# JosefAlbers/Phi-3-Vision-MLX

Measured on AMD Instinct MI355X. Metric: decode tokens/sec through generate()'s loop (reference-defined; bare graph replays: device_rate) + prefill ms, Phi-3-Vision bf16 1-image VQA, higher is better.
Workload: dtype bf16; 1 GPU; Phi-3-Vision single 336x336 image VQA (BASELINE configs[1]); 17 crops, 2509 image tokens + 22 text tokens, prompt 2531, B=1 per GPU, greedy, EOS suppressed; parallelism=batch-sharded replicas x1, batch_per_gpu=1, tiny=False

## Files before the change

### include/p3v.h

```cpp
#ifndef P3V_H
#define P3V_H
#include <stdint.h>

#ifdef __cplusplus
extern "C" {
#endif

#define P3V_VERSION 600
#define P3V_OK 0
#define P3V_ERR_ARG (-22)
#define P3V_ERR_LAUNCH (-5)
#define P3V_ERR_UNSUPPORTED (-95)
#define P3V_ERR_HIP (-14)

typedef struct {
  int cu_count, lds_per_cu, wave_size, clock_khz, mem_clock_khz, mem_bus_bits;
  int64_t hbm_bytes;
  char arch[32];
} p3v_props_t;

int p3v_version(void);
int p3v_device_props(int device, p3v_props_t* out );
const char* p3v_strerror(int code);

// ... 24 lines not shown
  const uint16_t* W;
  void* out;
  const uint16_t* bias;
  const void* resid;
  const uint16_t* pos;
  int M, N, K;
  int lda, ldw, ldo;
  int epilogue;
  int patches_per_img;
  void* ws;
  int64_t ws_bytes;
} p3v_gemm_args_t;
int p3v_gemm(const p3v_gemm_args_t* args , void* stream);
int64_t p3v_gemm_ws_bytes(int M, int N, int K, int epilogue);
int p3v_gemm_rows_slices(int M, int N, int K, int epilogue);

typedef struct {
  const uint16_t* x;
  const uint16_t* W;
  void* out;
  const uint16_t* resid;
  const uint16_t* norm_w;
  float norm_eps;
  int M, N, K;
  int epilogue;
} p3v_gemv_args_t;
int p3v_gemv(const p3v_gemv_args_t* args , void* stream);

typedef struct {
  const uint16_t* x; const uint8_t* W; const float* w_scale; void* out;
// ... 327 lines not shown
```

### phi-3-vision-mlx_amd/_lib.py

```python
import ctypes as C
import os

_HERE = os.path.dirname(os.path.abspath(__file__))
LIB_PATH = os.environ.get("P3V_LIB") or os.path.join(_HERE, "libp3v.so")

P3V_OK = 0
(EPI_NONE, EPI_BIAS, EPI_BIAS_QGELU, EPI_BIAS_GELU, EPI_BIAS_RESID_F32, EPI_RESID_BF16, EPI_SILU_MUL, EPI_PATCH,
 EPI_F32) = range(9)
DECODE_MAX_L = 16

vp, i32, i64, f32 = C.c_void_p, C.c_int, C.c_int64, C.c_float


class Props(C.Structure):
    _fields_ = [("cu_count", i32), ("lds_per_cu", i32), ("wave_size", i32), ("clock_khz", i32),
                ("mem_clock_khz", i32), ("mem_bus_bits", i32), ("hbm_bytes", i64), ("arch", C.c_char * 32)]


class GemmArgs(C.Structure):
    _fields_ = [("A", vp), ("W", vp), ("out", vp), ("bias", vp), ("resid", vp), ("pos", vp),
                ("M", i32), ("N", i32), ("K", i32), ("lda", i32), ("ldw", i32), ("ldo", i32),
                ("epilogue", i32), ("patches_per_img", i32), ("ws", vp), ("ws_bytes", i64)]


# ... 143 lines not shown
SAMPLE_MAX_N, SAMPLE_MAX_ROWS = 32768, 1024
POOL_LAST, POOL_MEAN = 0, 1
SIM_TOPK_MAX, SIM_TOPK_MAX_Q = 32, 16
SIGNATURES = {
    "p3v_version": (i32, []),
    "p3v_device_props": (i32, [i32, C.POINTER(Props)]),
    "p3v_strerror": (C.c_char_p, [i32]),
    "p3v_set_tuning": (i32, [C.c_char_p, i32]),
    "p3v_get_tuning": (i32, [C.c_char_p, C.POINTER(i32)]),
    "p3v_embed_gather": (i32, [vp, vp, vp, i32, i32, i32, vp]),
    "p3v_rmsnorm": (i32, [vp, vp, vp, i32, i32, f32, vp]),
    "p3v_layernorm": (i32, [vp, vp, vp, vp, i32, i32, i32, f32, vp]),
    "p3v_gemm": (i32, [C.POINTER(GemmArgs), vp]),
    "p3v_gemm_ws_bytes": (i64, [i32, i32, i32, i32]),
    "p3v_gemm_rows_slices": (i32, [i32, i32, i32, i32]),
    "p3v_gemv": (i32, [C.POINTER(GemvArgs), vp]),
    "p3v_gemv_step": (i32, [C.POINTER(GemvArgs), C.POINTER(GemvStep), vp]),
    "p3v_gemv_fp8_step": (i32, [C.POINTER(GemvF8Args), C.POINTER(GemvStep), vp]),
    "p3v_gemv_q4_step": (i32, [C.POINTER(GemvQ4Args), C.POINTER(GemvStep), vp]),
    "p3v_gemv_fp8": (i32, [C.POINTER(GemvF8Args), vp]),
    "p3v_dequant_fp8": (i32, [vp, vp, vp, i32, i32, vp]),
    "p3v_pack_b13": (i32, [vp, i32, i32, i32, vp, vp, vp]),
    "p3v_unpack_b13": (i32, [vp, i32, i32, i32, i32, vp, vp]),
    "p3v_gemv_b13": (i32, [C.POINTER(GemvB13Args), vp]),
    "p3v_gemv_b13_plan": (i32, [i32, i32, i32, i32, C.POINTER(i32)]),
    "p3v_gemv_b13_step": (i32, [C.POINTER(GemvB13Args), C.POINTER(GemvStep), vp]),
    "p3v_gemm_fp8": (i32, [C.POINTER(GemmF8Args), vp]),
    "p3v_quant_fp8_rows": (i32, [vp, vp, f32, vp, vp, i32, i32, vp]),
    "p3v_rope_table": (i32, [vp, vp, f32, vp, vp, i32, i32, vp]),
    "p3v_rope_kv_append": (i32, [vp, vp, vp, vp, vp, vp, i32, i32, i32, i32, i32, i32, vp, i32, i32, i32, i32, f32, vp]),
# ... 88 lines not shown
```

### phi-3-vision-mlx_amd/csrc/p3v_common.h

```cpp
#pragma once
#include <hip/hip_runtime.h>
#include <stdint.h>

#include "../../include/p3v.h"

typedef uint16_t bf16_t;
typedef __attribute__((ext_vector_type(8))) __bf16 bf16x8_t;
typedef __attribute__((ext_vector_type(4))) float f32x4_t;
typedef __attribute__((ext_vector_type(16))) float f32x16_t;
typedef __attribute__((ext_vector_type(4))) uint32_t u32x4_t;
typedef __attribute__((ext_vector_type(2))) uint32_t u32x2_t;

#define P3V_WAVE 64
#define P3V_MAX_DEVICES 64

#define P3V_CHECK_LAUNCH()                                   \
  do {                                                       \
    hipError_t e_ = hipGetLastError();                       \
    if (e_ != hipSuccess) return P3V_ERR_LAUNCH;             \
  } while (0)

__device__ __forceinline__ float bf16_to_f32(bf16_t u) { return __uint_as_float(((uint32_t)u) << 16); }

typedef __attribute__((ext_vector_type(2))) __bf16 bf16x2_t;
// ... 84 lines not shown
  float t = -INFINITY;
  for (int i = 0; i < nw; ++i) t = fmaxf(t, red[i]);
  return t;
}

static inline int p3v_cdiv(long a, long b) { return (int)((a + b - 1) / b); }
static inline int p3v_gemv_wpw(int waves, int n_cu, int forced) {
  if (forced == 3 || forced == 4) return forced;
  const float w3 = (float)p3v_cdiv(p3v_cdiv(waves, 3), n_cu) * 3.f * n_cu / (float)waves;
  const float w4 = (float)p3v_cdiv(p3v_cdiv(waves, 4), n_cu) * 4.f * n_cu / (float)waves;
  return w3 < w4 - 0.05f ? 3 : 4;
}

struct P3vTuning {
  int gemm_big_rows;
  int gemm_no_splitk, gemm_splitk_max_m, gemm_splitk_max_s, gemm_splitk_wgs, gemm_128, gemm_persistent;
  int gemm_rows;
  int gemm_no_skinny, gemm_skinny_max_m, gemm_skinny_s, gemm_skinny_tm128;
  int gemm_no_qkv_fuse;
  int gemm_f8_narrow;
  int attn_no_dma, attn_old, attn_pp, attn_il, attn_il_waves, combine_g, kvq_old, q8_old;
  int attn_fo_map_q8;
  int attn_fo_map;
  int gemv_no_mfma, gemv_no_mfma8, gemv_wpc, gemv8_wgs, gemv_variant, gemv_rows, gemv8_min, gemv_mfma8, gemv_f8_wpc, gemv_q4_wpc, gemv_wpw, gemv_q4_rows_wgs, gemv_q4_rows8;
  int gemv_b13_wpc, gemv_b13_wpc_end;
  int gemv_b13_xscale;
};
const P3vTuning& p3v_tuning();
```

### phi-3-vision-mlx_amd/csrc/p3v_gemm.hip

```cpp
#include <stdlib.h>
#include <string.h>


#include "p3v_gemm_qkv.h"

#define P3V_EPI_QKV 100

#define BM 128
#define BN 128
#define BK 64
#define TILE_BYTES (BM * BK * 2)
#define GEMM_LDS (4 * TILE_BYTES)

typedef const __attribute__((address_space(1))) void* gptr_t;
typedef __attribute__((address_space(3))) void* lptr_t;

struct GemmP {
  const bf16_t* A; const bf16_t* W; void* out; const bf16_t* bias; const void* resid; const bf16_t* pos;
  int M, N, K, lda, ldw, ldo, ppi;
  int kslice;
  QkvP q;
};

__device__ __forceinline__ float gelu_erf(float x) { return 0.5f * x * (1.f + erff(x * 0.70710678118654752f)); }
// ... 242 lines not shown
  if (!attr_set) {
    if (hipFuncSetAttribute((const void*)k_gemm<EPI, ORD>, hipFuncAttributeMaxDynamicSharedMemorySize, GEMM_LDS) != hipSuccess)
      return P3V_ERR_HIP;
    attr_set = true;
  }
  const int n_tile = EPI == P3V_EPI_SILU_MUL ? BN / 2 : BN;
  dim3 grid(p3v_cdiv(p.N, n_tile), p3v_cdiv(p.M, BM), p.kslice ? p.K / p.kslice : 1);
  hipLaunchKernelGGL((k_gemm<EPI, ORD>), grid, dim3(256), GEMM_LDS, s, p);
  P3V_CHECK_LAUNCH();
  return P3V_OK;
}

template <int EPI>
static int launch_gemm(const GemmP& p, hipStream_t s) { return launch_gemm_v<EPI, 0>(p, s); }

int p3v_gemm256_try(const p3v_gemm_args_t* a, hipStream_t s);
static int gemm128(const p3v_gemm_args_t* a, hipStream_t s);

static int gemm_big_rows(const p3v_gemm_args_t* a) {
  const int n_big = a->epilogue == P3V_EPI_SILU_MUL ? 128 : 256, n_small = n_big / 2;
  if (a->M < 1024 || a->N % n_big || a->epilogue == P3V_EPI_PATCH) return 0;
  if (const int force = p3v_tuning().gemm_big_rows; force >= 0) return min(force / 256 * 256, a->M);
  const int mt = p3v_cdiv(a->M, 256), nt_big = a->N / n_big, nt_small = p3v_cdiv(a->N, n_small);
  const float big_round = a->K >= 2048 ? 1.0f : 1.0f + 0.25f * (2048 - a->K) / 1024.f;
  float best = 1e30f;
  int best_rows = 0;
  for (int ms = 0; ms <= mt; ++ms) {
    const int rows_big = min(ms * 256, a->M), rows_small = a->M - rows_big;
    const long big = (long)ms * nt_big, small = (long)p3v_cdiv(rows_small, 128) * nt_small;
    float c = (float)((big + 255) / 256) * big_round;
    if (small) {
      const long full = small / 512, rest = small % 512;
      c += 0.675f * full + (rest == 0 ? 0.f : rest <= 256 ? 0.42f : 0.675f);
    }
    if (big && small) c += 0.04f;
    if (c < best - 1e-4f) { best = c; best_rows = rows_big; }
  }
  return best_rows;
}

template <int EPI>
__global__ void __launch_bounds__(256) k_splitk_reduce(const float* __restrict__ part, void* __restrict__ out, const void* __restrict__ resid,
                                                       int M, int N, int ldp, int ldo, int S) {
  constexpr bool SILU = EPI == P3V_EPI_SILU_MUL;
  const int per_row = N / 8;
  const long i = (long)blockIdx.x * 256 + threadIdx.x;
  if (i >= (long)M * per_row) return;
  const int m = (int)(i / per_row), n = (int)(i - (long)m * per_row) * 8;
  float v[8] = {0, 0, 0, 0, 0, 0, 0, 0}, u[8] = {0, 0, 0, 0, 0, 0, 0, 0};
  for (int z = 0; z < S; ++z) {
    const float* pr = part + ((size_t)z * M + m) * ldp + n;
    const float4 a0 = *(const float4*)pr, a1 = *(const float4*)(pr + 4);
    v[0] += a0.x; v[1] += a0.y; v[2] += a0.z; v[3] += a0.w; v[4] += a1.x; v[5] += a1.y; v[6] += a1.z; v[7] += a1.w;
// ... 152 lines not shown
  if (a->M == 0) return P3V_OK;
  {
    const size_t w_rows = (size_t)a->N * (a->epilogue == P3V_EPI_SILU_MUL ? 2 : 1);
    if ((size_t)a->M * a->lda * 2 >= (1ull << 32) || w_rows * a->ldw * 2 >= (1ull << 32)) return P3V_ERR_UNSUPPORTED;
  }
  hipStream_t s = (hipStream_t)stream;
  if (!a->bias) {
    const int rc = p3v_gemm_skinny_try(a, s);
    if (rc != P3V_ERR_UNSUPPORTED) return rc;
  }
  {
    const int rc = gemm_splitk(a, s);
    if (rc != P3V_ERR_UNSUPPORTED) return rc;
  }
  const bool big_tiles = !p3v_tuning().gemm_128;
  const int rows_big = big_tiles ? gemm_big_rows(a) : 0;
  if (rows_big > 0) {
    p3v_gemm_args_t top = *a;
    top.M = rows_big;
    const int rc = p3v_gemm256_try(&top, s);
    if (rc == P3V_OK && rows_big < a->M) {
      const bool f32_out = a->epilogue == P3V_EPI_BIAS_RESID_F32 || a->epilogue == P3V_EPI_F32;
      const size_t out_row = (size_t)a->ldo * (f32_out ? 4 : 2);
      p3v_gemm_args_t rest = *a;
      rest.M = a->M - rows_big;
      rest.A = a->A + (size_t)rows_big * a->lda;
      rest.out = (char*)a->out + rows_big * out_row;
      if (a->resid) rest.resid = (const char*)a->resid + rows_big * out_row;
      return gemm128(&rest, s);
    }
    if (rc != P3V_ERR_UNSUPPORTED) return rc;
  }
  return gemm128(a, s);
}

// ... 25 lines not shown
  if (sp->B <= 0 || sp->L <= 0 || nh <= 0 || nkv <= 0 || hd <= 0 || sp->tab_div <= 0 || !(sp->q_scale > 0.f)) return P3V_ERR_ARG;
  if (a->M != sp->B * sp->L || a->N != (nh + 2 * nkv) * hd || a->K % BK || a->lda < a->K || a->ldw < a->K || a->lda % 8 || a->ldw % 8) return P3V_ERR_ARG;
  if (((uintptr_t)a->A | (uintptr_t)a->W | (uintptr_t)a->bias | (uintptr_t)sp->q_out | (uintptr_t)sp->k_dst | (uintptr_t)sp->v_dst |
       (uintptr_t)sp->cos_t | (uintptr_t)sp->sin_t) & 15)
    return P3V_ERR_ARG;
  const int dpos0 = sp->dst_off_is_past ? sp->past : 0;
  if (hd % 32 || half % 16 || dpos0 % 8 || sp->dst_t % 8 || p3v_tuning().gemm_no_qkv_fuse) return P3V_ERR_UNSUPPORTED;
  if ((size_t)a->M * a->lda * 2 >= (1ull << 32) || (size_t)a->N * a->ldw * 2 >= (1ull << 32)) return P3V_ERR_UNSUPPORTED;
  hipStream_t s = (hipStream_t)stream;
  QkvP q = {sp->cos_t, sp->sin_t, sp->q_out, sp->k_dst, sp->v_dst, sp->L, nh, nkv, hd, sp->past, dpos0, sp->dst_t, sp->tab_t, sp->tab_div, 0,
            sp->q_scale};
  if (a->M < 1024) return p3v_gemm_skinny_qkv(a, q, s);
  if ((nh * hd) % BN || (nkv * hd) % BN || p3v_tuning().gemm_128) return P3V_ERR_UNSUPPORTED;
  p3v_gemm_args_t plain = *a;
  plain.epilogue = P3V_EPI_NONE;
  int rows_big = (nh * hd) % 256 || (nkv * hd) % 256 ? 0 : gemm_big_rows(&plain);
  if (rows_big > 0) {
    p3v_gemm_args_t top = *a;
    top.M = rows_big;
    const int rc = p3v_gemm256_qkv(&top, q, s);
    if (rc == P3V_ERR_UNSUPPORTED) rows_big = 0;
    else if (rc != P3V_OK) return rc;
  }
  if (rows_big < a->M) {
    q.m_base = rows_big;
    const GemmP p = {a->A + (size_t)rows_big * a->lda, a->W, nullptr, a->bias, nullptr, nullptr, a->M - rows_big, a->N, a->K, a->lda, a->ldw, 0, 0, 0, q};
    return launch_gemm<P3V_EPI_QKV>(p, s);
  }
  return P3V_OK;
}
```

### phi-3-vision-mlx_amd/csrc/p3v_gemm256.hip

```cpp
#include <stdlib.h>

#include "p3v_gemm256_epi.h"

#define BUF_BYTES (4 * HALF_BYTES)
#define GEMM256_LDS (2 * BUF_BYTES)

struct Tile256 {
  int m0, n0; int a_off[2][2], b_off[2][2]; __amdgpu_buffer_rsrc_t rs_a;
  int swapped, is_k, row0;
};

#ifdef P3V_G256_DEBUG
__device__ unsigned long long p3v_g256dbg[8 * 64 * 8];
#define G_S(k) do { __builtin_amdgcn_sched_barrier(0); asm volatile("s_memtime %0" : "=s"(g_s[k])); __builtin_amdgcn_sched_barrier(0); } while (0)
#define G_FLUSH(it) do { if (blockIdx.x == P3V_G256_DEBUG && (threadIdx.x & 63) == 0 && (it) < 64) { for (int k_ = 0; k_ < 8; ++k_) p3v_g256dbg[((threadIdx.x >> 6) * 64 + (it)) * 8 + k_] = g_s[k_]; } } while (0)
extern "C" int p3v_g256dbg_read(unsigned long long* out) {
  return hipMemcpyFromSymbol(out, HIP_SYMBOL(p3v_g256dbg), sizeof(unsigned long long) * 8 * 64 * 8) == hipSuccess ? 0 : -1;
}
#else
#define G_S(k) do { } while (0)
#define G_FLUSH(it) do { } while (0)
#endif
template <int EPI, int SCHED = 0x50, int ORDER = 0>
__global__ void __launch_bounds__(512, 1) k_gemm256(Gemm256P p) {
  constexpr bool SILU = EPI == P3V_EPI_SILU_MUL, QKV = EPI == P3V_EPI_QKV;
  extern __shared__ __attribute__((aligned(16))) unsigned char smem[];
  const int tid = threadIdx.x, lane = tid & 63, wave = __builtin_amdgcn_readfirstlane(tid >> 6);
  const int wr = wave >> 2, wc = wave & 3;
  constexpr int n_out_tile = SILU ? TN / 2 : TN;
  const int gx = (p.N + n_out_tile - 1) / n_out_tile, gy = (p.M + TM - 1) / TM, nwg = gx * gy;
  const int nq_t = QKV ? p.q.nh * p.q.hd / TN : 0, nk_t = QKV ? p.q.nkv * p.q.hd / TN : 0;

  using Tile = Tile256;
  const int srow = tid >> 3, schunk = tid & 7;
  auto make_tile = [&](int wid, Tile& t) {
    const int q = nwg >> 3, r = nwg & 7, xcd = wid & 7, loc = wid >> 3;
    const int id = (xcd < r ? xcd * (q + 1) : r * (q + 1) + (xcd - r) * q) + loc;
    constexpr int BAND = 4;
    const int band = id / (BAND * gx), in_band = id % (BAND * gx);
    const int rows = min(BAND, gy - band * BAND);
    const int m_t = band * BAND + in_band % rows, n_t = in_band / rows;
    t.m0 = m_t * TM, t.n0 = n_t * n_out_tile;
    t.swapped = t.is_k = t.row0 = 0;
    if (QKV) {
      t.swapped = n_t >= nq_t + nk_t;
      t.is_k = !t.swapped && n_t >= nq_t;
      t.row0 = t.swapped ? (p.q.nh + p.q.nkv) * p.q.hd : t.is_k ? p.q.nh * p.q.hd : 0;
      t.n0 = (n_t - (t.swapped ? nq_t + nk_t : t.is_k ? nq_t : 0)) * TN;
    }
#pragma unroll
    for (int h = 0; h < 2; ++h)
#pragma unroll
      for (int qq = 0; qq < 2; ++qq) {
        const int rr = h * 128 + qq * 64 + srow;
        const int sw = (schunk ^ (rr & 7)) * 8;
        const int ar = min(t.m0 + rr, p.M - 1) - t.m0;
        int br;
        if (SILU) {
          const int wcol = rr >> 6, ni = (rr & 63) >> 4, c = rr & 15;
          br = min(t.n0 + wcol * 32 + (ni & 1) * 16 + c, p.N - 1) + (ni >> 1) * p.N;
        } else if (QKV) {
          br = qkv_pair_row(p.q, t.row0, t.n0 >> 1, rr);
        } else {
          br = min(t.n0 + rr, p.N - 1);
        }
        if (QKV && t.swapped) {
          t.a_off[h][qq] = (rr * p.ldw + sw) * 2;
          t.b_off[h][qq] = (int)(((unsigned)(t.m0 + ar) * (unsigned)p.lda + (unsigned)sw) * 2u);
        } else {
          t.a_off[h][qq] = (ar * p.lda + sw) * 2;
          t.b_off[h][qq] = (int)(((unsigned)br * (unsigned)p.ldw + (unsigned)sw) * 2u);
        }
      }
    t.rs_a = QKV && t.swapped ? __builtin_amdgcn_make_buffer_rsrc((void*)(p.W + (size_t)(t.row0 + t.n0) * p.ldw), 0, 0xffffffff, 0x00020000)
                              : __builtin_amdgcn_make_buffer_rsrc((void*)(p.A + (size_t)t.m0 * p.lda), 0, 0xffffffff, 0x00020000);
  };
  const __amdgpu_buffer_rsrc_t rs_w = __builtin_amdgcn_make_buffer_rsrc((void*)p.W, 0, 0xffffffff, 0x00020000);
  const __amdgpu_buffer_rsrc_t rs_x = __builtin_amdgcn_make_buffer_rsrc((void*)p.A, 0, 0xffffffff, 0x00020000);
  auto dma_half = [&](const Tile& t, int which, int kt, int buf) {
    unsigned char* base = smem + buf * BUF_BYTES + which * HALF_BYTES + wave * 1024;
    const int h = which & 1;
#pragma unroll
    for (int q = 0; q < 2; ++q) {
      const __amdgpu_buffer_rsrc_t rs = which < 2 ? t.rs_a : (QKV && t.swapped) ? rs_x : rs_w;
      const int vo = which < 2 ? t.a_off[h][q] : t.b_off[h][q];
      __builtin_amdgcn_raw_ptr_buffer_load_lds(rs, (lptr_t)(base + q * 8192), 16, vo, kt * (TK * 2), 0, 0);
    }
  };

  const int frow = lane & 15, fchunk = lane >> 4;
  const int nk = p.K / TK;
  int wid = blockIdx.x;
  if (wid >= nwg) return;
  Tile cur_t;
  make_tile(wid, cur_t);
#pragma unroll
  for (int w4 = 0; w4 < 4; ++w4) dma_half(cur_t, w4, 0, 0);
  int gk = 0;
  bool landed = false;
  for (;;) {
  const int m0 = cur_t.m0, n0 = cur_t.n0;
  const bool has_next = wid + (int)gridDim.x < nwg;
  f32x4_t acc[8][4];
#pragma unroll
  for (int i = 0; i < 8; ++i)
#pragma unroll
    for (int j = 0; j < 4; ++j) acc[i][j] = (f32x4_t){0.f, 0.f, 0.f, 0.f};

#ifdef P3V_G256_DEBUG
  unsigned long long g_s[8] = {0, 0, 0, 0, 0, 0, 0, 0};
#endif
  for (int kt = 0; kt < nk; ++kt, ++gk) {
    G_S(0);
    if (!(kt == 0 && landed)) asm volatile("s_waitcnt vmcnt(0)" ::: "memory");
    G_S(1);
    __builtin_amdgcn_s_barrier();
    G_S(2);
    const bool last = kt + 1 == nk;
    const bool more = !last || has_next;
    const int nb = (gk + 1) & 1;
    const unsigned char* ta = smem + (gk & 1) * BUF_BYTES + wr * HALF_BYTES;
    const unsigned char* tb = smem + (gk & 1) * BUF_BYTES + (2 + (wc >> 1)) * HALF_BYTES + (wc & 1) * 64 * 128;
    bf16x8_t af[4][2], af1[4][2], bf0[2][2], bf1[2][2];
    auto read_a_to = [&](int sub, bf16x8_t (&dst)[4][2]) {
#pragma unroll
      for (int i = 0; i < 4; ++i)
#pragma unroll
        for (int kk = 0; kk < 2; ++kk) {
          const int r = sub * 64 + i * 16 + frow;
          dst[i][kk] = *(const bf16x8_t*)(ta + r * 128 + (((kk * 4 + fchunk) ^ (r & 7)) << 4));
        }
    };
    auto read_a = [&](int sub) { read_a_to(sub, af); };
    auto read_b = [&](int sub, bf16x8_t (&bf)[2][2]) {
#pragma unroll
      for (int j = 0; j < 2; ++j)
#pragma unroll
        for (int kk = 0; kk < 2; ++kk) {
          const int r = sub * 32 + j * 16 + frow;
          bf[j][kk] = *(const bf16x8_t*)(tb + r * 128 + (((kk * 4 + fchunk) ^ (r & 7)) << 4));
        }
    };
    auto quad_from = [&](int asub, int bsub, bf16x8_t (&a)[4][2], bf16x8_t (&bf)[2][2]) {
      __builtin_amdgcn_s_setprio(1);
#pragma unroll
      for (int kk = 0; kk < 2; ++kk)
#pragma unroll
        for (int i = 0; i < 4; ++i)
#pragma unroll
          for (int j = 0; j < 2; ++j)
            acc[asub * 4 + i][bsub * 2 + j] =
                __builtin_amdgcn_mfma_f32_16x16x32_bf16(bf[j][kk], a[i][kk], acc[asub * 4 + i][bsub * 2 + j], 0, 0, 0);
      __builtin_amdgcn_s_setprio(0);
    };
    auto quad = [&](int asub, int bsub, bf16x8_t (&bf)[2][2]) { quad_from(asub, bsub, af, bf); };
    auto dma_phase = [&](int ph) {
      if (more) {
#pragma unroll
        for (int h = 0; h < 4; ++h)
          if (((SCHED >> (2 * h)) & 3) == ph) {
            if (!last) dma_half(cur_t, h, kt + 1, nb);
            else {
              Tile nt;
              make_tile(wid + gridDim.x, nt);
              dma_half(nt, h, 0, nb);
            }
          }
// ... 35 lines not shown
    read_a(1);
    if (ORDER == 1) dma_phase(2);
    quad(1, 1, bf1);
    dma_phase(3);
    quad(1, 0, bf0);
  }

  if (has_next) {
    asm volatile("s_waitcnt vmcnt(0)" ::: "memory");
    landed = true;
  }
  if constexpr (QKV) {
    if (!cur_t.swapped) qkv_epilogue_rot<8>(p.q, acc, p.bias, cur_t.is_k, cur_t.row0, (n0 >> 1) + wc * 32, m0 + wr * 128, p.M, lane);
    else qkv_epilogue_vt<8>(p.q, acc, p.bias ? p.bias + cur_t.row0 : nullptr, n0 + wr * 128, m0 + wc * 64, p.M, lane);
  } else {
    gemm256_epilogue<EPI>(p, acc, m0, n0, wr, wc, lane);
  }
  if (!has_next) break;
  wid += gridDim.x;
  make_tile(wid, cur_t);
  }
}

template <int EPI, int SCHED, int ORDER>
static int launch_gemm256_v(const Gemm256P& p, hipStream_t s) {
  static bool attr_set = false;
  if (!attr_set) {
    if (hipFuncSetAttribute((const void*)k_gemm256<EPI, SCHED, ORDER>, hipFuncAttributeMaxDynamicSharedMemorySize, GEMM256_LDS) != hipSuccess)
      return P3V_ERR_HIP;
    attr_set = true;
  }
  const int n_tile = EPI == P3V_EPI_SILU_MUL ? TN / 2 : TN;
  static int n_cu = 0;
  if (!n_cu) {
    int dev = 0;
    hipDeviceProp_t pr;
    if (hipGetDevice(&dev) != hipSuccess || hipGetDeviceProperties(&pr, dev) != hipSuccess) return P3V_ERR_HIP;
    n_cu = pr.multiProcessorCount / 8 * 8;
  }
  const int tiles = p3v_cdiv(p.N, n_tile) * p3v_cdiv(p.M, TM);
  const int persist = p3v_tuning().gemm_persistent;
  dim3 grid(persist ? min(tiles, n_cu) : tiles);
  hipLaunchKernelGGL((k_gemm256<EPI, SCHED, ORDER>), grid, dim3(512), GEMM256_LDS, s, p);
  P3V_CHECK_LAUNCH();
  return P3V_OK;
}

template <int EPI>
static int launch_gemm256(const Gemm256P& p, hipStream_t s) { return launch_gemm256_v<EPI, 0x50, 2>(p, s); }

int p3v_gemm256_qkv(const p3v_gemm_args_t* a, const QkvP& q, hipStream_t s) {
  if (a->N % TN || a->K % TK || (q.nh * q.hd) % TN || (q.nkv * q.hd) % TN) return P3V_ERR_UNSUPPORTED;
  if ((size_t)a->N * a->ldw * 2 >= ((size_t)1 << 32) || (size_t)a->M * a->lda * 2 >= ((size_t)1 << 32)) return P3V_ERR_UNSUPPORTED;
  const Gemm256P p = {a->A, a->W, nullptr, a->bias, nullptr, a->M, a->N, a->K, a->lda, a->ldw, 0, q};
  return launch_gemm256<P3V_EPI_QKV>(p, s);
}

int p3v_gemm256_try(const p3v_gemm_args_t* a, hipStream_t s) {
  const int n_tile = a->epilogue == P3V_EPI_SILU_MUL ? TN / 2 : TN;
  if (a->N % n_tile || a->K % TK || a->epilogue == P3V_EPI_PATCH) return P3V_ERR_UNSUPPORTED;
  const size_t w_rows = (size_t)a->N * (a->epilogue == P3V_EPI_SILU_MUL ? 2 : 1);
  if (w_rows * a->ldw * 2 >= ((size_t)1 << 32) || (size_t)256 * a->lda * 2 >= ((size_t)1 << 31)) return P3V_ERR_UNSUPPORTED;
  const Gemm256P p = {a->A, a->W, a->out, a->bias, a->resid, a->M, a->N, a->K, a->lda, a->ldw, a->ldo, {}};
  switch (a->epilogue) {
    case P3V_EPI_NONE: return launch_gemm256<P3V_EPI_NONE>(p, s);
    case P3V_EPI_BIAS: return launch_gemm256<P3V_EPI_BIAS>(p, s);
    case P3V_EPI_BIAS_QGELU: return launch_gemm256<P3V_EPI_BIAS_QGELU>(p, s);
    case P3V_EPI_BIAS_GELU: return launch_gemm256<P3V_EPI_BIAS_GELU>(p, s);
    case P3V_EPI_BIAS_RESID_F32: return launch_gemm256<P3V_EPI_BIAS_RESID_F32>(p, s);
    case P3V_EPI_RESID_BF16: return launch_gemm256<P3V_EPI_RESID_BF16>(p, s);
    case P3V_EPI_SILU_MUL: return launch_gemm256<P3V_EPI_SILU_MUL>(p, s);
    case P3V_EPI_F32: return launch_gemm256<P3V_EPI_F32>(p, s);
    default: return P3V_ERR_UNSUPPORTED;
  }
}
```

### phi-3-vision-mlx_amd/csrc/p3v_gemm256_epi.h

```cpp
#pragma once
#include "p3v_gemm_qkv.h"

#define P3V_EPI_QKV 100

#define TM 256
#define TN 256
#define TK 64
#define HALF_BYTES (128 * TK * 2)

typedef const __attribute__((address_space(1))) void* gptr_t;
typedef __attribute__((address_space(3))) void* lptr_t;

struct Gemm256P {
  const bf16_t* A; const bf16_t* W; void* out; const bf16_t* bias; const void* resid;
  int M, N, K, lda, ldw, ldo;
  QkvP q;
};

__device__ __forceinline__ float gelu_erf2(float x) { return 0.5f * x * (1.f + erff(x * 0.70710678118654752f)); }

template <int EPI>
__device__ __forceinline__ void gemm256_epilogue(const Gemm256P& p, f32x4_t (&acc)[8][4], int m0, int n0, int wr, int wc, int lane) {
  constexpr bool SILU = EPI == P3V_EPI_SILU_MUL;
  const int fc = lane & 15, fq = lane >> 4;
  const int mrow0 = m0 + wr * 128 + fc;
#if defined(P3V_G256_ABL) && P3V_G256_ABL == 3
#pragma unroll
  for (int i = 0; i < 8; ++i)
#pragma unroll
    for (int j = 0; j < 4; ++j) asm volatile("" :: "v"(acc[i][j]));
#else
  if (SILU) {
    const int n = n0 + wc * 32 + (fq & 1) * 16 + (fq >> 1) * 8;
#pragma unroll
    for (int i = 0; i < 8; ++i) {
      uint32_t pk[2][2];
#pragma unroll
      for (int j = 0; j < 2; ++j) {
        float o4[4];
#pragma unroll
        for (int r = 0; r < 4; ++r) {
          const float g = bf16_round(acc[i][j][r]), u = bf16_round(acc[i][2 + j][r]);
          o4[r] = bf16_round(g * bf16_round(1.f / (1.f + __expf(-g)))) * u;
        }
        pk[j][0] = pack_bf16x2(o4[0], o4[1]), pk[j][1] = pack_bf16x2(o4[2], o4[3]);
      }
      u32x4_t w;
#pragma unroll
      for (int k = 0; k < 2; ++k) {
        auto sw = __builtin_amdgcn_permlane16_swap(pk[0][k], pk[1][k], false, false);
        w[k] = sw[0], w[2 + k] = sw[1];
      }
      const int m = mrow0 + i * 16;
      if (m < p.M && n < p.N) *(u32x4_t*)((bf16_t*)p.out + (size_t)m * p.ldo + n) = w;
    }
  } else if (EPI == P3V_EPI_BIAS_RESID_F32 || EPI == P3V_EPI_F32) {
    float bias[4][4];
#pragma unroll
    for (int j = 0; j < 4; ++j) {
      const int n = n0 + wc * 64 + j * 16 + fq * 4;
      u32x2_t bw = {0u, 0u};
      if (p.bias && n < p.N) bw = *(const u32x2_t*)(p.bias + n);
      bias[j][0] = bf16lo(bw[0]), bias[j][1] = bf16hi(bw[0]), bias[j][2] = bf16lo(bw[1]), bias[j][3] = bf16hi(bw[1]);
    }
#pragma unroll
    for (int i = 0; i < 8; ++i) {
      const int m = mrow0 + i * 16;
#pragma unroll
      for (int j = 0; j < 4; ++j) {
        const int n = n0 + wc * 64 + j * 16 + fq * 4;
        if (m < p.M && n < p.N) {
          const size_t o = (size_t)m * p.ldo + n;
          float4 v = make_float4(acc[i][j][0] + bias[j][0], acc[i][j][1] + bias[j][1], acc[i][j][2] + bias[j][2], acc[i][j][3] + bias[j][3]);
          if (EPI == P3V_EPI_BIAS_RESID_F32) {
            const float4 r4 = *(const float4*)((const float*)p.resid + o);
            v.x += r4.x, v.y += r4.y, v.z += r4.z, v.w += r4.w;
          }
          *(float4*)((float*)p.out + o) = v;
        }
      }
    }
  } else {
    float bias[4][4];
#pragma unroll
    for (int j = 0; j < 4; ++j) {
      const int n = n0 + wc * 64 + j * 16 + fq * 4;
      u32x2_t bw = {0u, 0u};
      if (p.bias && n < p.N) bw = *(const u32x2_t*)(p.bias + n);
      bias[j][0] = bf16lo(bw[0]), bias[j][1] = bf16hi(bw[0]), bias[j][2] = bf16lo(bw[1]), bias[j][3] = bf16hi(bw[1]);
    }
#pragma unroll
    for (int i = 0; i < 8; ++i) {
      const int m = mrow0 + i * 16;
#pragma unroll
      for (int jp = 0; jp < 2; ++jp) {
        uint32_t pk[2][2];
#pragma unroll
        for (int jj = 0; jj < 2; ++jj) {
          const int j = 2 * jp + jj;
          float v[4];
#pragma unroll
          for (int r = 0; r < 4; ++r) {
            v[r] = acc[i][j][r] + bias[j][r];
            if (EPI == P3V_EPI_BIAS_QGELU) v[r] = v[r] * p3v_sigmoid(1.702f * v[r]);
            else if (EPI == P3V_EPI_BIAS_GELU) v[r] = gelu_erf2(v[r]);
          }
          pk[jj][0] = pack_bf16x2(v[0], v[1]), pk[jj][1] = pack_bf16x2(v[2], v[3]);
// ... 27 lines not shown
```

### phi-3-vision-mlx_amd/csrc/p3v_runtime.hip

```cpp
#include <ctype.h>
#include <stdlib.h>
#include <string.h>

#include <mutex>

#include "p3v_common.h"

extern "C" int p3v_version(void) { return P3V_VERSION; }

extern "C" const char* p3v_strerror(int code) {
  switch (code) {
    case P3V_OK: return "ok";
    case P3V_ERR_ARG: return "invalid argument (shape, alignment or null pointer)";
    case P3V_ERR_LAUNCH: return "kernel launch failed";
    case P3V_ERR_UNSUPPORTED: return "unsupported combination";
    case P3V_ERR_HIP: return "HIP runtime call failed";
    default: return "unknown error";
  }
}

namespace {
struct Knob { const char* name; int P3vTuning::*field; int dflt; };
const Knob kKnobs[] = {
    {"gemm_big_rows", &P3vTuning::gemm_big_rows, -1},       {"gemm_no_splitk", &P3vTuning::gemm_no_splitk, 0},
// ... 4 lines not shown
    {"attn_old", &P3vTuning::attn_old, 0},                  {"attn_pp", &P3vTuning::attn_pp, -1},
    {"attn_il", &P3vTuning::attn_il, -1},                   {"attn_il_waves", &P3vTuning::attn_il_waves, -1},
                      {"combine_g", &P3vTuning::combine_g, -1},
    {"kvq_old", &P3vTuning::kvq_old, 0},                    {"q8_old", &P3vTuning::q8_old, 0},
    {"gemv_no_mfma", &P3vTuning::gemv_no_mfma, 0},          {"gemv_no_mfma8", &P3vTuning::gemv_no_mfma8, 0},
    {"gemv_wpc", &P3vTuning::gemv_wpc, 8},                  {"gemv8_wgs", &P3vTuning::gemv8_wgs, 256},
    {"gemv_variant", &P3vTuning::gemv_variant, 3},          {"gemv_rows", &P3vTuning::gemv_rows, 1},
    {"gemv8_min", &P3vTuning::gemv8_min, 2},                {"gemv_mfma8", &P3vTuning::gemv_mfma8, 1},
    {"gemv_f8_wpc", &P3vTuning::gemv_f8_wpc, 16},           {"gemv_q4_wpc", &P3vTuning::gemv_q4_wpc, 8},
    {"gemv_wpw", &P3vTuning::gemv_wpw, 0},                  {"gemv_q4_rows_wgs", &P3vTuning::gemv_q4_rows_wgs, 256},
    {"gemv_q4_rows8", &P3vTuning::gemv_q4_rows8, 1},
    {"gemv_b13_wpc", &P3vTuning::gemv_b13_wpc, 16},         {"gemv_b13_wpc_end", &P3vTuning::gemv_b13_wpc_end, 8},
    {"gemv_b13_xscale", &P3vTuning::gemv_b13_xscale, 1},
    {"gemm_no_skinny", &P3vTuning::gemm_no_skinny, 0},     {"gemm_skinny_max_m", &P3vTuning::gemm_skinny_max_m, 256},
    {"gemm_skinny_s", &P3vTuning::gemm_skinny_s, 0},            {"gemm_skinny_tm128", &P3vTuning::gemm_skinny_tm128, 0},
    {"gemm_rows", &P3vTuning::gemm_rows, 1},
    {"attn_fo_map", &P3vTuning::attn_fo_map, 2},              {"attn_fo_map_q8", &P3vTuning::attn_fo_map_q8, 0},
};
P3vTuning g_tuning;
std::once_flag g_tuning_once;
void tuning_init() {
  for (const Knob& k : kKnobs) {
    char env[64] = "P3V_";
    size_t n = 4;
    for (const char* c = k.name; *c && n + 1 < sizeof(env); ++c) env[n++] = (char)toupper((unsigned char)*c);
    env[n] = 0;
    const char* e = getenv(env);
    g_tuning.*(k.field) = !e ? k.dflt : !strcmp(e, "auto") ? -1 : (*e == 0 ? 1 : atoi(e));
  }
}
}
// ... 83 lines not shown
```

### phi-3-vision-mlx_amd/ops.py

```python
import collections
import contextlib
import ctypes as C
import weakref

import numpy as np
import torch

from . import _lib as L
from ._lib import (EPI_BIAS, EPI_BIAS_GELU, EPI_BIAS_QGELU, EPI_BIAS_RESID_F32, EPI_F32, EPI_NONE,
                   EPI_PATCH, EPI_RESID_BF16, EPI_SILU_MUL)

BF16, F32, I32 = torch.bfloat16, torch.float32, torch.int32


def _stream():
    return torch.cuda.current_stream().cuda_stream


def _p(t):
    return 0 if t is None else t.data_ptr()


def _chk(t, dtype, name):
    if not t.is_cuda:
# ... 304 lines not shown
    out = torch.empty((pk.rows, pk.K), dtype=BF16, device=pk.data.device) if out is None else out
    L.check(L.lib().p3v_unpack_b13(_p(pk.data), pk.rows, pk.K, int(pk.silu_pairs), pk.base, _p(out), _stream()), "unpack_b13")
    return out


def gemv_b13(x, pk, epilogue=EPI_NONE, resid=None, norm_w=None, norm_eps=0.0, out=None):
    _chk(x, BF16, "x")
    rc, out = _gemv_launch("gemv_b13", _B13, pk, x, x.shape[0], epilogue, resid, norm_w, norm_eps, out)
    L.check(rc, "gemv_b13")
    return out


def gemv_b13_plan(N, K, epilogue, n_cu):
    out = (C.c_int32 * 4)()
    L.check(L.lib().p3v_gemv_b13_plan(int(N), int(K), int(epilogue), int(n_cu), out), "gemv_b13_plan")
    return tuple(out)


def dequant_fp8(w8, w_scale, out=None):
    N, K = w8.shape
    out = torch.empty((N, K), dtype=BF16, device=w8.device) if out is None else out
    L.check(L.lib().p3v_dequant_fp8(_p(w8), _p(w_scale), _p(out), N, K, _stream()), "dequant_fp8")
    return out


def quant_fp8_rows(x, norm_w=None, norm_eps=0.0, out=None, scale=None):
    _chk(x, BF16, "x")
    M, K = x.shape
    out = torch.empty((M, K), dtype=torch.uint8, device=x.device) if out is None else out
    scale = torch.empty((M,), dtype=F32, device=x.device) if scale is None else scale
# ... 622 lines not shown
```

Measured before the change: 578.4 tokens/s.

## Add 192- and 128-row tile heights to gemm256 with a cost-model planner

Templates the 256-row GEMM kernel on the number of row blocks so it can also run 192- and 128-row tiles, skipping the unused A-tile loads. A new planner scores each tile height and big/small row split against the CU count and picks the cheapest, which aims to cut tail-wave waste on prefill GEMMs. It also exposes the planner through the C API and Python and adds a tuning knob to pin the height. This only affects prefill GEMMs, so decode throughput should barely change. The shorter tiles do less MFMA work per load, and the heuristic cost constants may choose poorly.

```diff
diff --git a/include/p3v.h b/include/p3v.h
--- a/include/p3v.h
+++ b/include/p3v.h
@@ -62,6 +62,7 @@
 int p3v_gemm(const p3v_gemm_args_t* args , void* stream);
 int64_t p3v_gemm_ws_bytes(int M, int N, int K, int epilogue);
 int p3v_gemm_rows_slices(int M, int N, int K, int epilogue);
+int p3v_gemm_plan(int M, int N, int K, int epilogue, int n_cu, int* out );
 
 typedef struct {
   const uint16_t* x;
diff --git a/phi-3-vision-mlx_amd/_lib.py b/phi-3-vision-mlx_amd/_lib.py
--- a/phi-3-vision-mlx_amd/_lib.py
+++ b/phi-3-vision-mlx_amd/_lib.py
@@ -181,6 +181,7 @@
     "p3v_gemm": (i32, [C.POINTER(GemmArgs), vp]),
     "p3v_gemm_ws_bytes": (i64, [i32, i32, i32, i32]),
     "p3v_gemm_rows_slices": (i32, [i32, i32, i32, i32]),
+    "p3v_gemm_plan": (i32, [i32, i32, i32, i32, i32, C.POINTER(i32)]),
     "p3v_gemv": (i32, [C.POINTER(GemvArgs), vp]),
     "p3v_gemv_step": (i32, [C.POINTER(GemvArgs), C.POINTER(GemvStep), vp]),
     "p3v_gemv_fp8_step": (i32, [C.POINTER(GemvF8Args), C.POINTER(GemvStep), vp]),
diff --git a/phi-3-vision-mlx_amd/csrc/p3v_common.h b/phi-3-vision-mlx_amd/csrc/p3v_common.h
--- a/phi-3-vision-mlx_amd/csrc/p3v_common.h
+++ b/phi-3-vision-mlx_amd/csrc/p3v_common.h
@@ -122,6 +122,7 @@
 
 struct P3vTuning {
   int gemm_big_rows;
+  int gemm_tile_rows;
   int gemm_no_splitk, gemm_splitk_max_m, gemm_splitk_max_s, gemm_splitk_wgs, gemm_128, gemm_persistent;
   int gemm_rows;
   int gemm_no_skinny, gemm_skinny_max_m, gemm_skinny_s, gemm_skinny_tm128;
diff --git a/phi-3-vision-mlx_amd/csrc/p3v_gemm.hip b/phi-3-vision-mlx_amd/csrc/p3v_gemm.hip
--- a/phi-3-vision-mlx_amd/csrc/p3v_gemm.hip
+++ b/phi-3-vision-mlx_amd/csrc/p3v_gemm.hip
@@ -280,29 +280,55 @@
 template <int EPI>
 static int launch_gemm(const GemmP& p, hipStream_t s) { return launch_gemm_v<EPI, 0>(p, s); }
 
-int p3v_gemm256_try(const p3v_gemm_args_t* a, hipStream_t s);
+int p3v_gemm256_try(const p3v_gemm_args_t* a, int tile_rows, hipStream_t s);
 static int gemm128(const p3v_gemm_args_t* a, hipStream_t s);
 
-static int gemm_big_rows(const p3v_gemm_args_t* a) {
-  const int n_big = a->epilogue == P3V_EPI_SILU_MUL ? 128 : 256, n_small = n_big / 2;
-  if (a->M < 1024 || a->N % n_big || a->epilogue == P3V_EPI_PATCH) return 0;
-  if (const int force = p3v_tuning().gemm_big_rows; force >= 0) return min(force / 256 * 256, a->M);
-  const int mt = p3v_cdiv(a->M, 256), nt_big = a->N / n_big, nt_small = p3v_cdiv(a->N, n_small);
-  const float big_round = a->K >= 2048 ? 1.0f : 1.0f + 0.25f * (2048 - a->K) / 1024.f;
+struct GemmPlan { int tile, rows; };
+
+constexpr float GEMM_ROUND_192 = 0.09f, GEMM_ROUND_128 = 0.23f;
+static GemmPlan gemm_plan(int M, int N, int K, int epilogue, int n_cu, int heights) {
+  const int n_big = epilogue == P3V_EPI_SILU_MUL ? 128 : 256, n_small = n_big / 2;
+  if (M < 1024 || N % n_big || epilogue == P3V_EPI_PATCH) return {256, 0};
+  const P3vTuning& tu = p3v_tuning();
+  const int pin = tu.gemm_tile_rows;
+  if (heights & 6) heights = pin == 256 ? 1 : pin == 192 ? 2 : pin == 128 ? 4 : heights;
+  if (const int force = tu.gemm_big_rows; force >= 0) {
+    const int h = heights & 1 ? 256 : heights & 2 ? 192 : 128;
+    return {h, min(force / h * h, M)};
+  }
+  const int nt_big = N / n_big, nt_small = p3v_cdiv(N, n_small);
+  const float big_round = K >= 2048 ? 1.0f : 1.0f + 0.25f * (2048 - K) / 1024.f;
   float best = 1e30f;
-  int best_rows = 0;
-  for (int ms = 0; ms <= mt; ++ms) {
-    const int rows_big = min(ms * 256, a->M), rows_small = a->M - rows_big;
-    const long big = (long)ms * nt_big, small = (long)p3v_cdiv(rows_small, 128) * nt_small;
-    float c = (float)((big + 255) / 256) * big_round;
-    if (small) {
-      const long full = small / 512, rest = small % 512;
-      c += 0.675f * full + (rest == 0 ? 0.f : rest <= 256 ? 0.42f : 0.675f);
-    }
-    if (big && small) c += 0.04f;
-    if (c < best - 1e-4f) { best = c; best_rows = rows_big; }
-  }
-  return best_rows;
+  GemmPlan plan = {256, 0};
+  for (int hi = 0; hi < 3; ++hi) {
+    if (!(heights >> hi & 1)) continue;
+    const int h = 256 - 64 * hi;
+    const float round = hi == 0 ? big_round : big_round * h / 256.f + (hi == 1 ? GEMM_ROUND_192 : GEMM_ROUND_128);
+    const int mt = p3v_cdiv(M, h);
+    for (int ms = 0; ms <= mt; ++ms) {
+      const int rows_big = min(ms * h, M), rows_small = M - rows_big;
+      const long big = (long)ms * nt_big, small = (long)p3v_cdiv(rows_small, 128) * nt_small;
+      float c = (float)((big + n_cu - 1) / n_cu) * round;
+      if (small) {
+        const long full = small / (2 * n_cu), rest = small % (2 * n_cu);
+        c += 0.675f * full + (rest == 0 ? 0.f : rest <= n_cu ? 0.42f : 0.675f);
+      }
+      if (big && small) c += 0.04f;
+      if (c < best - 1e-4f) { best = c; plan = {h, rows_big}; }
+    }
+  }
+  return plan;
+}
+static GemmPlan gemm_plan(const p3v_gemm_args_t* a, int heights) { return gemm_plan(a->M, a->N, a->K, a->epilogue, 256, heights); }
+
+extern "C" int p3v_gemm_plan(int M, int N, int K, int epilogue, int n_cu, int* out) {
+  if (!out || M <= 0 || N <= 0 || K <= 0 || n_cu <= 0 || epilogue < 0 || epilogue > P3V_EPI_F32) return P3V_ERR_ARG;
+  const GemmPlan pl = gemm_plan(M, N, K, epilogue, n_cu, 7);
+  const int n_tile = epilogue == P3V_EPI_SILU_MUL ? 128 : 256;
+  out[0] = pl.tile, out[1] = pl.rows;
+  out[2] = pl.rows ? min(p3v_cdiv(pl.rows, pl.tile) * p3v_cdiv(N, n_tile), n_cu) : 0;
+  out[3] = M - pl.rows;
+  return P3V_OK;
 }
 
 template <int EPI>
@@ -485,11 +511,12 @@
     if (rc != P3V_ERR_UNSUPPORTED) return rc;
   }
   const bool big_tiles = !p3v_tuning().gemm_128;
-  const int rows_big = big_tiles ? gemm_big_rows(a) : 0;
+  const GemmPlan plan = big_tiles ? gemm_plan(a, 7) : GemmPlan{256, 0};
+  const int rows_big = plan.rows;
   if (rows_big > 0) {
     p3v_gemm_args_t top = *a;
     top.M = rows_big;
-    const int rc = p3v_gemm256_try(&top, s);
+    const int rc = p3v_gemm256_try(&top, plan.tile, s);
     if (rc == P3V_OK && rows_big < a->M) {
       const bool f32_out = a->epilogue == P3V_EPI_BIAS_RESID_F32 || a->epilogue == P3V_EPI_F32;
       const size_t out_row = (size_t)a->ldo * (f32_out ? 4 : 2);
@@ -545,7 +572,7 @@
   if ((nh * hd) % BN || (nkv * hd) % BN || p3v_tuning().gemm_128) return P3V_ERR_UNSUPPORTED;
   p3v_gemm_args_t plain = *a;
   plain.epilogue = P3V_EPI_NONE;
-  int rows_big = (nh * hd) % 256 || (nkv * hd) % 256 ? 0 : gemm_big_rows(&plain);
+  int rows_big = (nh * hd) % 256 || (nkv * hd) % 256 ? 0 : gemm_plan(&plain, 1).rows;
   if (rows_big > 0) {
     p3v_gemm_args_t top = *a;
     top.M = rows_big;
diff --git a/phi-3-vision-mlx_amd/csrc/p3v_gemm256.hip b/phi-3-vision-mlx_amd/csrc/p3v_gemm256.hip
--- a/phi-3-vision-mlx_amd/csrc/p3v_gemm256.hip
+++ b/phi-3-vision-mlx_amd/csrc/p3v_gemm256.hip
@@ -21,14 +21,16 @@
 #define G_S(k) do { } while (0)
 #define G_FLUSH(it) do { } while (0)
 #endif
-template <int EPI, int SCHED = 0x50, int ORDER = 0>
+template <int EPI, int SCHED = 0x50, int ORDER = 0, int MB = 8>
 __global__ void __launch_bounds__(512, 1) k_gemm256(Gemm256P p) {
   constexpr bool SILU = EPI == P3V_EPI_SILU_MUL, QKV = EPI == P3V_EPI_QKV;
+  static_assert(MB == 8 || ((MB == 6 || MB == 4) && !QKV), "tile heights: 256, 192, 128 rows; the qkv epilogue keeps 256");
+  constexpr int TMH = 32 * MB, HROWS = 16 * MB, HB = MB / 2;
   extern __shared__ __attribute__((aligned(16))) unsigned char smem[];
   const int tid = threadIdx.x, lane = tid & 63, wave = __builtin_amdgcn_readfirstlane(tid >> 6);
   const int wr = wave >> 2, wc = wave & 3;
   constexpr int n_out_tile = SILU ? TN / 2 : TN;
-  const int gx = (p.N + n_out_tile - 1) / n_out_tile, gy = (p.M + TM - 1) / TM, nwg = gx * gy;
+  const int gx = (p.N + n_out_tile - 1) / n_out_tile, gy = (p.M + TMH - 1) / TMH, nwg = gx * gy;
   const int nq_t = QKV ? p.q.nh * p.q.hd / TN : 0, nk_t = QKV ? p.q.nkv * p.q.hd / TN : 0;
 
   using Tile = Tile256;
@@ -40,7 +42,7 @@
     const int band = id / (BAND * gx), in_band = id % (BAND * gx);
     const int rows = min(BAND, gy - band * BAND);
     const int m_t = band * BAND + in_band % rows, n_t = in_band / rows;
-    t.m0 = m_t * TM, t.n0 = n_t * n_out_tile;
+    t.m0 = m_t * TMH, t.n0 = n_t * n_out_tile;
     t.swapped = t.is_k = t.row0 = 0;
     if (QKV) {
       t.swapped = n_t >= nq_t + nk_t;
@@ -54,7 +56,8 @@
       for (int qq = 0; qq < 2; ++qq) {
         const int rr = h * 128 + qq * 64 + srow;
         const int sw = (schunk ^ (rr & 7)) * 8;
-        const int ar = min(t.m0 + rr, p.M - 1) - t.m0;
+        const int ra = HROWS == 128 ? rr : h * HROWS + qq * 64 + srow;
+        const int ar = min(t.m0 + ra, p.M - 1) - t.m0;
         int br;
         if (SILU) {
           const int wcol = rr >> 6, ni = (rr & 63) >> 4, c = rr & 15;
@@ -82,6 +85,7 @@
     const int h = which & 1;
 #pragma unroll
     for (int q = 0; q < 2; ++q) {
+      if (q == 1 && which < 2 && (HROWS <= 64 || (HROWS < 128 && wave >= (HROWS - 64) / 8))) continue;
       const __amdgpu_buffer_rsrc_t rs = which < 2 ? t.rs_a : (QKV && t.swapped) ? rs_x : rs_w;
       const int vo = which < 2 ? t.a_off[h][q] : t.b_off[h][q];
       __builtin_amdgcn_raw_ptr_buffer_load_lds(rs, (lptr_t)(base + q * 8192), 16, vo, kt * (TK * 2), 0, 0);
@@ -101,9 +105,9 @@
   for (;;) {
   const int m0 = cur_t.m0, n0 = cur_t.n0;
   const bool has_next = wid + (int)gridDim.x < nwg;
-  f32x4_t acc[8][4];
-#pragma unroll
-  for (int i = 0; i < 8; ++i)
+  f32x4_t acc[MB][4];
+#pragma unroll
+  for (int i = 0; i < MB; ++i)
 #pragma unroll
     for (int j = 0; j < 4; ++j) acc[i][j] = (f32x4_t){0.f, 0.f, 0.f, 0.f};
 
@@ -121,13 +125,13 @@
     const int nb = (gk + 1) & 1;
     const unsigned char* ta = smem + (gk & 1) * BUF_BYTES + wr * HALF_BYTES;
     const unsigned char* tb = smem + (gk & 1) * BUF_BYTES + (2 + (wc >> 1)) * HALF_BYTES + (wc & 1) * 64 * 128;
-    bf16x8_t af[4][2], af1[4][2], bf0[2][2], bf1[2][2];
-    auto read_a_to = [&](int sub, bf16x8_t (&dst)[4][2]) {
-#pragma unroll
-      for (int i = 0; i < 4; ++i)
+    bf16x8_t af[HB][2], af1[HB][2], bf0[2][2], bf1[2][2];
+    auto read_a_to = [&](int sub, bf16x8_t (&dst)[HB][2]) {
+#pragma unroll
+      for (int i = 0; i < HB; ++i)
 #pragma unroll
         for (int kk = 0; kk < 2; ++kk) {
-          const int r = sub * 64 + i * 16 + frow;
+          const int r = sub * (16 * HB) + i * 16 + frow;
           dst[i][kk] = *(const bf16x8_t*)(ta + r * 128 + (((kk * 4 + fchunk) ^ (r & 7)) << 4));
         }
     };
@@ -141,16 +145,16 @@
           bf[j][kk] = *(const bf16x8_t*)(tb + r * 128 + (((kk * 4 + fchunk) ^ (r & 7)) << 4));
         }
     };
-    auto quad_from = [&](int asub, int bsub, bf16x8_t (&a)[4][2], bf16x8_t (&bf)[2][2]) {
+    auto quad_from = [&](int asub, int bsub, bf16x8_t (&a)[HB][2], bf16x8_t (&bf)[2][2]) {
       __builtin_amdgcn_s_setprio(1);
 #pragma unroll
       for (int kk = 0; kk < 2; ++kk)
 #pragma unroll
-        for (int i = 0; i < 4; ++i)
+        for (int i = 0; i < HB; ++i)
 #pragma unroll
           for (int j = 0; j < 2; ++j)
-            acc[asub * 4 + i][bsub * 2 + j] =
-                __builtin_amdgcn_mfma_f32_16x16x32_bf16(bf[j][kk], a[i][kk], acc[asub * 4 + i][bsub * 2 + j], 0, 0, 0);
+            acc[asub * HB + i][bsub * 2 + j] =
+                __builtin_amdgcn_mfma_f32_16x16x32_bf16(bf[j][kk], a[i][kk], acc[asub * HB + i][bsub * 2 + j], 0, 0, 0);
       __builtin_amdgcn_s_setprio(0);
     };
     auto quad = [&](int asub, int bsub, bf16x8_t (&bf)[2][2]) { quad_from(asub, bsub, af, bf); };
@@ -216,7 +220,7 @@
     if (!cur_t.swapped) qkv_epilogue_rot<8>(p.q, acc, p.bias, cur_t.is_k, cur_t.row0, (n0 >> 1) + wc * 32, m0 + wr * 128, p.M, lane);
     else qkv_epilogue_vt<8>(p.q, acc, p.bias ? p.bias + cur_t.row0 : nullptr, n0 + wr * 128, m0 + wc * 64, p.M, lane);
   } else {
-    gemm256_epilogue<EPI>(p, acc, m0, n0, wr, wc, lane);
+    gemm256_epilogue<EPI, MB>(p, acc, m0, n0, wr, wc, lane);
   }
   if (!has_next) break;
   wid += gridDim.x;
@@ -224,11 +228,11 @@
   }
 }
 
-template <int EPI, int SCHED, int ORDER>
+template <int EPI, int SCHED, int ORDER, int MB>
 static int launch_gemm256_v(const Gemm256P& p, hipStream_t s) {
   static bool attr_set = false;
   if (!attr_set) {
-    if (hipFuncSetAttribute((const void*)k_gemm256<EPI, SCHED, ORDER>, hipFuncAttributeMaxDynamicSharedMemorySize, GEMM256_LDS) != hipSuccess)
+    if (hipFuncSetAttribute((const void*)k_gemm256<EPI, SCHED, ORDER, MB>, hipFuncAttributeMaxDynamicSharedMemorySize, GEMM256_LDS) != hipSuccess)
       return P3V_ERR_HIP;
     attr_set = true;
   }
@@ -240,39 +244,49 @@
     if (hipGetDevice(&dev) != hipSuccess || hipGetDeviceProperties(&pr, dev) != hipSuccess) return P3V_ERR_HIP;
     n_cu = pr.multiProcessorCount / 8 * 8;
   }
-  const int tiles = p3v_cdiv(p.N, n_tile) * p3v_cdiv(p.M, TM);
+  const int tiles = p3v_cdiv(p.N, n_tile) * p3v_cdiv(p.M, 32 * MB);
   const int persist = p3v_tuning().gemm_persistent;
   dim3 grid(persist ? min(tiles, n_cu) : tiles);
-  hipLaunchKernelGGL((k_gemm256<EPI, SCHED, ORDER>), grid, dim3(512), GEMM256_LDS, s, p);
+  hipLaunchKernelGGL((k_gemm256<EPI, SCHED, ORDER, MB>), grid, dim3(512), GEMM256_LDS, s, p);
   P3V_CHECK_LAUNCH();
   return P3V_OK;
 }
 
+#ifndef P3V_G256_SCHED_SHORT
+#define P3V_G256_SCHED_SHORT 0x50
+#endif
 template <int EPI>
-static int launch_gemm256(const Gemm256P& p, hipStream_t s) { return launch_gemm256_v<EPI, 0x50, 2>(p, s); }
+static int launch_gemm256(const Gemm256P& p, int tile_rows, hipStream_t s) {
+  if constexpr (EPI != P3V_EPI_QKV) {
+    if (tile_rows == 192) return launch_gemm256_v<EPI, P3V_G256_SCHED_SHORT, 2, 6>(p, s);
+    if (tile_rows == 128) return launch_gemm256_v<EPI, P3V_G256_SCHED_SHORT, 2, 4>(p, s);
+  }
+  if (tile_rows != TM) return P3V_ERR_UNSUPPORTED;
+  return launch_gemm256_v<EPI, 0x50, 2, 8>(p, s);
+}
 
 int p3v_gemm256_qkv(const p3v_gemm_args_t* a, const QkvP& q, hipStream_t s) {
   if (a->N % TN || a->K % TK || (q.nh * q.hd) % TN || (q.nkv * q.hd) % TN) return P3V_ERR_UNSUPPORTED;
   if ((size_t)a->N * a->ldw * 2 >= ((size_t)1 << 32) || (size_t)a->M * a->lda * 2 >= ((size_t)1 << 32)) return P3V_ERR_UNSUPPORTED;
   const Gemm256P p = {a->A, a->W, nullptr, a->bias, nullptr, a->M, a->N, a->K, a->lda, a->ldw, 0, q};
-  return launch_gemm256<P3V_EPI_QKV>(p, s);
-}
-
-int p3v_gemm256_try(const p3v_gemm_args_t* a, hipStream_t s) {
+  return launch_gemm256<P3V_EPI_QKV>(p, TM, s);
+}
+
+int p3v_gemm256_try(const p3v_gemm_args_t* a, int tile_rows, hipStream_t s) {
   const int n_tile = a->epilogue == P3V_EPI_SILU_MUL ? TN / 2 : TN;
   if (a->N % n_tile || a->K % TK || a->epilogue == P3V_EPI_PATCH) return P3V_ERR_UNSUPPORTED;
   const size_t w_rows = (size_t)a->N * (a->epilogue == P3V_EPI_SILU_MUL ? 2 : 1);
   if (w_rows * a->ldw * 2 >= ((size_t)1 << 32) || (size_t)256 * a->lda * 2 >= ((size_t)1 << 31)) return P3V_ERR_UNSUPPORTED;
   const Gemm256P p = {a->A, a->W, a->out, a->bias, a->resid, a->M, a->N, a->K, a->lda, a->ldw, a->ldo, {}};
   switch (a->epilogue) {
-    case P3V_EPI_NONE: return launch_gemm256<P3V_EPI_NONE>(p, s);
-    case P3V_EPI_BIAS: return launch_gemm256<P3V_EPI_BIAS>(p, s);
-    case P3V_EPI_BIAS_QGELU: return launch_gemm256<P3V_EPI_BIAS_QGELU>(p, s);
-    case P3V_EPI_BIAS_GELU: return launch_gemm256<P3V_EPI_BIAS_GELU>(p, s);
-    case P3V_EPI_BIAS_RESID_F32: return launch_gemm256<P3V_EPI_BIAS_RESID_F32>(p, s);
-    case P3V_EPI_RESID_BF16: return launch_gemm256<P3V_EPI_RESID_BF16>(p, s);
-    case P3V_EPI_SILU_MUL: return launch_gemm256<P3V_EPI_SILU_MUL>(p, s);
-    case P3V_EPI_F32: return launch_gemm256<P3V_EPI_F32>(p, s);
+    case P3V_EPI_NONE: return launch_gemm256<P3V_EPI_NONE>(p, tile_rows, s);
+    case P3V_EPI_BIAS: return launch_gemm256<P3V_EPI_BIAS>(p, tile_rows, s);
+    case P3V_EPI_BIAS_QGELU: return launch_gemm256<P3V_EPI_BIAS_QGELU>(p, tile_rows, s);
+    case P3V_EPI_BIAS_GELU: return launch_gemm256<P3V_EPI_BIAS_GELU>(p, tile_rows, s);
+    case P3V_EPI_BIAS_RESID_F32: return launch_gemm256<P3V_EPI_BIAS_RESID_F32>(p, tile_rows, s);
+    case P3V_EPI_RESID_BF16: return launch_gemm256<P3V_EPI_RESID_BF16>(p, tile_rows, s);
+    case P3V_EPI_SILU_MUL: return launch_gemm256<P3V_EPI_SILU_MUL>(p, tile_rows, s);
+    case P3V_EPI_F32: return launch_gemm256<P3V_EPI_F32>(p, tile_rows, s);
     default: return P3V_ERR_UNSUPPORTED;
   }
 }
diff --git a/phi-3-vision-mlx_amd/csrc/p3v_gemm256_epi.h b/phi-3-vision-mlx_amd/csrc/p3v_gemm256_epi.h
--- a/phi-3-vision-mlx_amd/csrc/p3v_gemm256_epi.h
+++ b/phi-3-vision-mlx_amd/csrc/p3v_gemm256_epi.h
@@ -19,21 +19,21 @@
 
 __device__ __forceinline__ float gelu_erf2(float x) { return 0.5f * x * (1.f + erff(x * 0.70710678118654752f)); }
 
-template <int EPI>
-__device__ __forceinline__ void gemm256_epilogue(const Gemm256P& p, f32x4_t (&acc)[8][4], int m0, int n0, int wr, int wc, int lane) {
+template <int EPI, int MB = 8>
+__device__ __forceinline__ void gemm256_epilogue(const Gemm256P& p, f32x4_t (&acc)[MB][4], int m0, int n0, int wr, int wc, int lane) {
   constexpr bool SILU = EPI == P3V_EPI_SILU_MUL;
   const int fc = lane & 15, fq = lane >> 4;
-  const int mrow0 = m0 + wr * 128 + fc;
+  const int mrow0 = m0 + wr * (16 * MB) + fc;
 #if defined(P3V_G256_ABL) && P3V_G256_ABL == 3
 #pragma unroll
-  for (int i = 0; i < 8; ++i)
+  for (int i = 0; i < MB; ++i)
 #pragma unroll
     for (int j = 0; j < 4; ++j) asm volatile("" :: "v"(acc[i][j]));
 #else
   if (SILU) {
     const int n = n0 + wc * 32 + (fq & 1) * 16 + (fq >> 1) * 8;
 #pragma unroll
-    for (int i = 0; i < 8; ++i) {
+    for (int i = 0; i < MB; ++i) {
       uint32_t pk[2][2];
 #pragma unroll
       for (int j = 0; j < 2; ++j) {
@@ -64,7 +64,7 @@
       bias[j][0] = bf16lo(bw[0]), bias[j][1] = bf16hi(bw[0]), bias[j][2] = bf16lo(bw[1]), bias[j][3] = bf16hi(bw[1]);
     }
 #pragma unroll
-    for (int i = 0; i < 8; ++i) {
+    for (int i = 0; i < MB; ++i) {
       const int m = mrow0 + i * 16;
 #pragma unroll
       for (int j = 0; j < 4; ++j) {
@@ -90,7 +90,7 @@
       bias[j][0] = bf16lo(bw[0]), bias[j][1] = bf16hi(bw[0]), bias[j][2] = bf16lo(bw[1]), bias[j][3] = bf16hi(bw[1]);
     }
 #pragma unroll
-    for (int i = 0; i < 8; ++i) {
+    for (int i = 0; i < MB; ++i) {
       const int m = mrow0 + i * 16;
 #pragma unroll
       for (int jp = 0; jp < 2; ++jp) {
diff --git a/phi-3-vision-mlx_amd/csrc/p3v_runtime.hip b/phi-3-vision-mlx_amd/csrc/p3v_runtime.hip
--- a/phi-3-vision-mlx_amd/csrc/p3v_runtime.hip
+++ b/phi-3-vision-mlx_amd/csrc/p3v_runtime.hip
@@ -42,7 +42,7 @@
     {"gemv_b13_xscale", &P3vTuning::gemv_b13_xscale, 1},
     {"gemm_no_skinny", &P3vTuning::gemm_no_skinny, 0},     {"gemm_skinny_max_m", &P3vTuning::gemm_skinny_max_m, 256},
     {"gemm_skinny_s", &P3vTuning::gemm_skinny_s, 0},            {"gemm_skinny_tm128", &P3vTuning::gemm_skinny_tm128, 0},
-    {"gemm_rows", &P3vTuning::gemm_rows, 1},
+    {"gemm_rows", &P3vTuning::gemm_rows, 1},                {"gemm_tile_rows", &P3vTuning::gemm_tile_rows, -1},
     {"attn_fo_map", &P3vTuning::attn_fo_map, 2},              {"attn_fo_map_q8", &P3vTuning::attn_fo_map_q8, 0},
 };
 P3vTuning g_tuning;
diff --git a/phi-3-vision-mlx_amd/ops.py b/phi-3-vision-mlx_amd/ops.py
--- a/phi-3-vision-mlx_amd/ops.py
+++ b/phi-3-vision-mlx_amd/ops.py
@@ -342,6 +342,12 @@
 def gemv_b13_plan(N, K, epilogue, n_cu):
     out = (C.c_int32 * 4)()
     L.check(L.lib().p3v_gemv_b13_plan(int(N), int(K), int(epilogue), int(n_cu), out), "gemv_b13_plan")
+    return tuple(out)
+
+
+def gemm_plan(M, N, K, epilogue, n_cu=256):
+    out = (C.c_int32 * 4)()
+    L.check(L.lib().p3v_gemm_plan(int(M), int(N), int(K), int(epilogue), int(n_cu), out), "gemm_plan")
     return tuple(out)
 
 
```

Result: no change. 580.4 tokens/s, median of 4 (+0.3%).
